# lithium0003/findtextCenterNet

Hardware: AMD Instinct MI355X
Metric: 768x768 images/s (detector fwd+NMS) (higher is better)
Workload: dtype bf16; 1 GPU; BASELINE configs[1]: batch=8/GPU synthetic 768x768x3 uniform-noise tiles, full EfficientNetV2-XL detector forward + NMS + GPU peak decode/100-d gather; global_batch=8, tile=768x768x3, weights=deterministic seed 0 (random-init), parallelism=dp1

## Files before the change

findtextcenternet_amd/csrc/backbone_ops.hip:

```cpp
#include "ftc_common.h"
#include "ftc_host.h"

namespace {

template <typename OutT, typename CopyT, int NQ, bool FAST>
__global__ __launch_bounds__(256) void stem_kernel(const float* __restrict__ in, const float* __restrict__ w,
                                                   const float* __restrict__ bias, OutT* __restrict__ out, CopyT* __restrict__ out2,
                                                   int B, int H, int W, int Ho, int Wo, int C0, int nchw, int act) {
    extern __shared__ __attribute__((aligned(16))) float sw[];
    for (int i = threadIdx.x; i < 27 * C0; i += blockDim.x) sw[i] = w[i];
    __syncthreads();
    const int CG = C0 / (4 * NQ);
    const unsigned total = (unsigned)B * Ho * Wo * CG;
    for (unsigned idx = blockIdx.x * blockDim.x + threadIdx.x; idx < total; idx += gridDim.x * blockDim.x) {
        const unsigned pix = idx / (unsigned)CG;
        const int c0 = (int)(idx - pix * CG) * 4 * NQ;
        const unsigned row = pix / (unsigned)Wo;
        const int ox = (int)(pix - row * Wo);
        const int b = (int)(row / (unsigned)Ho);
        const int oy = (int)(row - (unsigned)b * Ho);
        f32x4 acc[NQ];
#pragma unroll
        for (int q = 0; q < NQ; ++q) acc[q] = *reinterpret_cast<const f32x4*>(bias + c0 + 4 * q);
#pragma unroll
        for (int r = 0; r < 3; ++r) {
            const int iy = oy * 2 - 1 + r;
#pragma unroll
            for (int s = 0; s < 3; ++s) {
                const int ix = ox * 2 - 1 + s;
                if ((unsigned)iy < (unsigned)H && (unsigned)ix < (unsigned)W) {
#pragma unroll
                    for (int c = 0; c < 3; ++c) {
                        const float v = nchw ? in[(((long)b * 3 + c) * H + iy) * W + ix]
                                             : in[(((long)b * H + iy) * W + ix) * 3 + c];
                        const float xv = v * 2.0f - 1.0f;
#pragma unroll
                        for (int q = 0; q < NQ; ++q) acc[q] += xv * *reinterpret_cast<const f32x4*>(sw + ((r * 3 + s) * 3 + c) * C0 + c0 + 4 * q);
                    }
                }
            }
        }
#pragma unroll
        for (int q = 0; q < NQ; ++q) {
            if (act) {
                if constexpr (FAST) acc[q] = act_silu_fast4(acc[q]);
                else {
#pragma unroll
                    for (int e = 0; e < 4; ++e) acc[q][e] = act_silu_precise(acc[q][e]);
                }
            }
            store4<OutT>(out + (long)pix * C0 + c0 + 4 * q, acc[q]);
            if (out2) store4<CopyT>(out2 + (long)pix * C0 + c0 + 4 * q, acc[q]);
        }
    }
}

template <typename T, int STRIDE>
__global__ __launch_bounds__(256) void dwconv_kernel(const T* __restrict__ in, const float* __restrict__ w,
                                                     const float* __restrict__ bias, T* __restrict__ out,
                                                     float* __restrict__ partial, int H, int W, int Ho, int Wo,
                                                     int C, int tilesX, int P, int tiles_per_wg, int act) {
    constexpr int V = 16 / (int)sizeof(T);
    constexpr int LPP = 64 / V;
    constexpr int SLOTS = 256 / LPP;
    constexpr int TH = STRIDE == 1 ? 8 : 4;
    constexpr int TW = 8;
    constexpr int IH = (TH - 1) * STRIDE + 3;
    constexpr int IW = (TW - 1) * STRIDE + 3;
    constexpr int NPX = IH * IW;
    constexpr int NLD = (NPX + SLOTS - 1) / SLOTS;
    __shared__ __attribute__((aligned(16))) T tile[2][NPX * 64];
    __shared__ __attribute__((aligned(16))) float red[SLOTS * 64];

    auto swz = [](int i) { return (STRIDE == 2 && sizeof(T) == 2) ? (i * 64) ^ (((i >> 1) & 1) << 6) : i * 64; };
    const int t = threadIdx.x;
    const int cq = t % LPP;
    const int pt = t / LPP;
    const int c = blockIdx.x * 64 + cq * V;
    const int b = blockIdx.z;
    const bool cok = c < C;
    const int tile0 = blockIdx.y * tiles_per_wg;
    const int ntile = min(tiles_per_wg, P - tile0);

    u32x4 stage[NLD];
    auto fetch = [&](int tileId) {
        const int ty = tileId / tilesX, tx = tileId - ty * tilesX;
        const int iy0 = ty * TH * STRIDE - 1, ix0 = tx * TW * STRIDE - 1;
#pragma unroll
        for (int j = 0; j < NLD; ++j) {
            const int i = pt + j * SLOTS;
            const int ry = i / IW, rx = i - ry * IW;
            const int iy = iy0 + ry, ix = ix0 + rx;
            u32x4 v = {0u, 0u, 0u, 0u};
            if (cok && i < NPX && (unsigned)iy < (unsigned)H && (unsigned)ix < (unsigned)W)
                v = *reinterpret_cast<const u32x4*>(in + (((long)b * H + iy) * W + ix) * C + c);
            stage[j] = v;
        }
    };
    auto commit = [&](int buf) {
#pragma unroll
        for (int j = 0; j < NLD; ++j) {
            const int i = pt + j * SLOTS;
            if (i < NPX) *reinterpret_cast<u32x4*>(&tile[buf][swz(i) + cq * V]) = stage[j];
        }
    };

    fetch(tile0);
    float wv[9][V], bv[V];
#pragma unroll
    for (int e = 0; e < V; ++e) bv[e] = 0.f;
#pragma unroll
    for (int k = 0; k < 9; ++k)
#pragma unroll
        for (int e = 0; e < V; ++e) wv[k][e] = 0.f;
    if (cok) {
#pragma unroll
        for (int k = 0; k < 9; ++k)
#pragma unroll
            for (int q = 0; q < V / 4; ++q) {
                const f32x4 x = *reinterpret_cast<const f32x4*>(w + (long)k * C + c + 4 * q);
#pragma unroll
                for (int e = 0; e < 4; ++e) wv[k][4 * q + e] = x[e];
            }
#pragma unroll
        for (int q = 0; q < V / 4; ++q) {
            const f32x4 x = *reinterpret_cast<const f32x4*>(bias + c + 4 * q);
#pragma unroll
            for (int e = 0; e < 4; ++e) bv[4 * q + e] = x[e];
        }
    }
    commit(0);
    __syncthreads();

    for (int kt = 0; kt < ntile; ++kt) {
        const int tileId = tile0 + kt;
        const int buf = kt & 1;
        if (kt + 1 < ntile) fetch(tileId + 1);
        const int ty = tileId / tilesX, tx = tileId - ty * tilesX;
        const int oy0 = ty * TH, ox0 = tx * TW;
        float sum[V];
#pragma unroll
        for (int e = 0; e < V; ++e) sum[e] = 0.f;
#pragma unroll
        for (int k = 0; k < TH * TW / SLOTS; ++k) {
            const int o = pt + SLOTS * k;
            const int ly = o / TW, lx = o - ly * TW;
            const int oy = oy0 + ly, ox = ox0 + lx;
            float acc[V];
#pragma unroll
            for (int e = 0; e < V; ++e) acc[e] = bv[e];
#pragma unroll
            for (int r = 0; r < 3; ++r)
#pragma unroll
                for (int s = 0; s < 3; ++s) {
                    float x[V];
                    load16<T>(&tile[buf][swz((ly * STRIDE + r) * IW + lx * STRIDE + s) + cq * V], x);
#pragma unroll
                    for (int e = 0; e < V; ++e) acc[e] = fmaf(wv[r * 3 + s][e], x[e], acc[e]);
                }
            if (cok && oy < Ho && ox < Wo) {
                if (act) {
#pragma unroll
                    for (int e = 0; e < V; ++e) acc[e] = sizeof(T) == 2 ? act_silu_fast(acc[e]) : act_silu_precise(acc[e]);
                }
                store16<T>(out + (((long)b * Ho + oy) * Wo + ox) * C + c, acc);
#pragma unroll
                for (int e = 0; e < V; ++e) sum[e] += acc[e];
            }
        }
#pragma unroll
        for (int e = 0; e < V; ++e) red[pt * 64 + cq * V + e] = sum[e];
        if (kt + 1 < ntile) commit(buf ^ 1);
        __syncthreads();
        if (t < 64) {
            float s = 0.f;
#pragma unroll
            for (int k = 0; k < SLOTS; ++k) s += red[k * 64 + t];
            const int cc = blockIdx.x * 64 + t;
            if (cc < C) partial[((long)b * P + tileId) * C + cc] = s;
        }
        __syncthreads();
    }
}

typedef __attribute__((address_space(3))) void lds_ptr_t;
__device__ __forceinline__ void dma16(__amdgpu_buffer_rsrc_t r, lds_ptr_t* dst, int voff) {
    __builtin_amdgcn_raw_ptr_buffer_load_lds(r, dst, 16, voff, 0, 0, 0);
}

template <typename T, bool PRECISE>
__global__ __launch_bounds__(256) void dwconv_strip_kernel(const T* __restrict__ in, const float* __restrict__ w,
                                                           const float* __restrict__ bias, T* __restrict__ out,
                                                           float* __restrict__ partial, int H, int W, int C, int tilesX,
                                                           int P, int tiles_per_wg, int act) {
    constexpr int TH = 8, TW = 8, IW = 10, NPX = 100;
    constexpr int CHS = 16 / (int)sizeof(T);
    constexpr int LPS = 64 / CHS;
    constexpr int PPW = 64 / LPS;
    constexpr int PPP = 4 * PPW;
    constexpr int NLD = (NPX + PPP - 1) / PPP;
    constexpr int OOB = 0x7ffffff0;
    __shared__ __attribute__((aligned(16))) T tile[2][NLD * PPP * 64];
    __shared__ __attribute__((aligned(16))) float red[16 * 64];

    const int t = threadIdx.x;
    const int b = blockIdx.z;
    const int c0 = blockIdx.x * 64;
    const int lane = t & 63, wave = __builtin_amdgcn_readfirstlane(t >> 6);
    const __amdgpu_buffer_rsrc_t rin = __builtin_amdgcn_make_buffer_rsrc(const_cast<T*>(in + (long)b * H * W * C), 0,
                                                                         H * W * C * (int)sizeof(T), 0x00020000);
    const int s_px = wave * PPW + lane / LPS;
    const int s_coff = (c0 + (lane % LPS) * CHS < C) ? (c0 + (lane % LPS) * CHS) * (int)sizeof(T) : OOB;
    const int cq = t & 15, col = (t >> 4) & 7, rh = t >> 7;
    const int c = c0 + cq * 4;
    const bool cok = c < C;
    const int tile0 = blockIdx.y * tiles_per_wg;
    const int ntile = min(tiles_per_wg, P - tile0);

    auto issue = [&](int tileId, int buf) {
        const int ty = tileId / tilesX, tx = tileId - ty * tilesX;
        const int iy0 = ty * TH - 1, ix0 = tx * TW - 1;
#pragma unroll
        for (int j = 0; j < NLD; ++j) {
            const int i = s_px + j * PPP;
            const int ry = i / IW, rx = i - ry * IW;
            const int iy = iy0 + ry, ix = ix0 + rx;
            const bool ok = i < NPX && (unsigned)iy < (unsigned)H && (unsigned)ix < (unsigned)W;
            dma16(rin, (lds_ptr_t*)&tile[buf][(j * PPP + wave * PPW) * 64], ok ? (iy * W + ix) * C * (int)sizeof(T) + s_coff : OOB);
        }
    };

    issue(tile0, 0);
    f32x4 wv[9], bv = {0.f, 0.f, 0.f, 0.f};
#pragma unroll
    for (int k = 0; k < 9; ++k) wv[k] = bv;
    if (cok) {
#pragma unroll
        for (int k = 0; k < 9; ++k) wv[k] = *reinterpret_cast<const f32x4*>(w + (long)k * C + c);
        bv = *reinterpret_cast<const f32x4*>(bias + c);
    }

    f32x4 sum = {0.f, 0.f, 0.f, 0.f};
    for (int kt = 0; kt < ntile; ++kt) {
        const int tileId = tile0 + kt;
        const int buf = kt & 1;
        asm volatile("s_waitcnt vmcnt(0)" ::: "memory");
        __syncthreads();
        if (kt + 1 < ntile) issue(tileId + 1, buf ^ 1);
        const int ty = tileId / tilesX, tx = tileId - ty * tilesX;
        const int oy0 = ty * TH + rh * 4, ox = tx * TW + col;
        f32x4 acc[4] = {bv, bv, bv, bv};
        const T* tp = &tile[buf][((rh * 4) * IW + col) * 64 + cq * 4];
#pragma unroll
        for (int r = 0; r < 6; ++r) {
            f32x4 x[3];
#pragma unroll
            for (int s2 = 0; s2 < 3; ++s2) x[s2] = load4<T>(tp + (r * IW + s2) * 64);
#pragma unroll
            for (int oo = 0; oo < 4; ++oo) {
                const int kr = r - oo;
                if (kr >= 0 && kr < 3) {
#pragma unroll
                    for (int s2 = 0; s2 < 3; ++s2)
#pragma unroll
                        for (int e = 0; e < 4; ++e) acc[oo][e] = fmaf(wv[kr * 3 + s2][e], x[s2][e], acc[oo][e]);
                }
            }
        }
#pragma unroll
        for (int oo = 0; oo < 4; ++oo) {
            const int oy = oy0 + oo;
            if (cok && oy < H && ox < W) {
                if (!PRECISE || act) {
#pragma unroll
                    for (int e = 0; e < 4; ++e) acc[oo][e] = PRECISE ? act_silu_precise(acc[oo][e]) : act_silu_fast(acc[oo][e]);
                }
                store4<T>(out + (((long)b * H + oy) * W + ox) * C + c, acc[oo]);
                sum += acc[oo];
            }
        }
    }
    *reinterpret_cast<f32x4*>(&red[(t >> 4) * 64 + cq * 4]) = sum;
    __syncthreads();
    if (t < 64 && c0 + t < C) {
        float s2 = 0.f;
#pragma unroll
        for (int k = 0; k < 16; ++k) s2 += red[k * 64 + t];
        float* pp = partial + ((long)b * P + tile0) * C + c0 + t;
        pp[0] = s2;
        for (int kt = 1; kt < ntile; ++kt) pp[(long)kt * C] = 0.f;
    }
}

__global__ __launch_bounds__(512) void se_fc1_kernel(const float* __restrict__ partial, const float* __restrict__ w1,
                                                     const float* __restrict__ b1, float* __restrict__ hidden,
                                                     int C, int S, int P, float inv_hw) {
    extern __shared__ __attribute__((aligned(16))) float mean[];
    const int b = blockIdx.y;
    const int t = threadIdx.x;
    const int CQ = C >> 2;
    const int lane = t & 63, wave = t >> 6;
    const int sidx = blockIdx.x * 8 + wave;
    constexpr int WMAX = 15;
    f32x4 wv[WMAX];
    const f32x4* wr = reinterpret_cast<const f32x4*>(w1 + (long)(sidx < S ? sidx : 0) * C);
#pragma unroll
    for (int i = 0; i < WMAX; ++i) {
        const int q = lane + 64 * i;
        wv[i] = q < CQ ? wr[q] : f32x4{0.f, 0.f, 0.f, 0.f};
    }
    const f32x4* pb = reinterpret_cast<const f32x4*>(partial + (long)b * P * C);
    for (int q = t; q < CQ; q += 512) {
        f32x4 s = {0.f, 0.f, 0.f, 0.f};
#pragma unroll 4
        for (int p = 0; p < P; ++p) s += pb[(long)p * CQ + q];
        reinterpret_cast<f32x4*>(mean)[q] = s * inv_hw;
    }
    __syncthreads();
    if (sidx >= S) return;
    f32x4 acc = {0.f, 0.f, 0.f, 0.f};
#pragma unroll
    for (int i = 0; i < WMAX; ++i) {
        const int q = lane + 64 * i;
        if (q < CQ) acc += wv[i] * reinterpret_cast<const f32x4*>(mean)[q];
    }
    for (int q = lane + 64 * WMAX; q < CQ; q += 64) acc += wr[q] * reinterpret_cast<const f32x4*>(mean)[q];
    float a = wave_sum((acc[0] + acc[1]) + (acc[2] + acc[3]));
    if (lane == 0) hidden[(long)b * S + sidx] = act_silu_precise(a + b1[sidx]);
}

__device__ __forceinline__ void se_load_hidden(float* hid, const float* __restrict__ hidden, const float* __restrict__ hpart,
                                               const float* __restrict__ b1, int b, int S, int NS, int t, int nthreads) {
    if (hpart) {
        const float* hp = hpart + (long)b * NS * S;
        for (int s = t; s < S; s += nthreads) {
            float a0 = 0.f, a1 = 0.f, a2 = 0.f, a3 = 0.f;
            int j = 0;
            for (; j + 4 <= NS; j += 4) {
                a0 += hp[(long)j * S + s];
                a1 += hp[(long)(j + 1) * S + s];
                a2 += hp[(long)(j + 2) * S + s];
                a3 += hp[(long)(j + 3) * S + s];
            }
            for (; j < NS; ++j) a0 += hp[(long)j * S + s];
            hid[s] = act_silu_precise(((a0 + a1) + (a2 + a3)) + b1[s]);
        }
    } else {
        for (int s = t; s < S; s += nthreads) hid[s] = hidden[(long)b * S + s];
    }
}

template <bool FOLD, typename T>
__global__ __launch_bounds__(256) void se_fc2_kernel(const float* __restrict__ hidden, const float* __restrict__ w2t,
                                                     const float* __restrict__ b2, float* __restrict__ scale, int C, int S,
                                                     const T* __restrict__ wp, T* __restrict__ wb, int N,
                                                     const float* __restrict__ hpart, const float* __restrict__ b1, int NS) {
    extern __shared__ __attribute__((aligned(16))) float hid[];
    const int b = blockIdx.y;
    se_load_hidden(hid, hidden, hpart, b1, b, S, NS, threadIdx.x, 256);
    __syncthreads();
    const int c = blockIdx.x * 256 + threadIdx.x;
    float sc = 0.f;
    if (c < C) {
        float acc = b2[c];
#pragma unroll 8
        for (int s = 0; s < S; ++s) acc += hid[s] * w2t[(long)s * C + c];
        sc = sigmoid_precise(acc);
        if (!FOLD || blockIdx.z == 0) scale[(long)b * C + c] = sc;
    }
    if constexpr (FOLD) {
        float* lsc = hid + S;
        lsc[threadIdx.x] = sc;
        __syncthreads();
        const int chunk = threadIdx.x & 31, r0 = threadIdx.x >> 5;
        const int cc = blockIdx.x * 256 + chunk * 8;
        if (cc >= C) return;
        float f[8];
#pragma unroll
        for (int e = 0; e < 8; ++e) f[e] = lsc[chunk * 8 + e];
        const int rows = (N + gridDim.z - 1) / gridDim.z;
        const int n_lo = blockIdx.z * rows, n_hi = min(N, n_lo + rows);
        T* dst = wb + (long)b * N * C;
#pragma unroll 4
        for (int n = n_lo + r0; n < n_hi; n += 8) {
            float x[8];
            load16<T>(wp + (long)n * C + cc, x);
#pragma unroll
            for (int e = 0; e < 8; ++e) x[e] *= f[e];
            store16<T>(dst + (long)n * C + cc, x);
        }
    }
}


template <typename T>
__global__ __launch_bounds__(256) void se_fc2_fold64_kernel(const float* __restrict__ hidden, const float* __restrict__ w2t,
                                                            const float* __restrict__ b2, float* __restrict__ scale, int C, int S,
                                                            const T* __restrict__ wp, T* __restrict__ wb, int N,
                                                            const float* __restrict__ hpart, const float* __restrict__ b1, int NS) {
    extern __shared__ __attribute__((aligned(16))) float lds_f[];
    float* hid = lds_f;
    float* part = lds_f + ((S + 3) & ~3);
    float* lsc = part + 256;
    const int b = blockIdx.y, t = threadIdx.x;
    const int cl = t & 63, sg = t >> 6;
    const int c = blockIdx.x * 64 + cl;
    const int s_lo = sg * ((S + 3) / 4), s_hi = min(S, s_lo + (S + 3) / 4);
    constexpr int SMAX = 40;
    float wreg[SMAX];
#pragma unroll
    for (int i = 0; i < SMAX; ++i) wreg[i] = (c < C && s_lo + i < s_hi) ? w2t[(long)(s_lo + i) * C + c] : 0.f;
    se_load_hidden(hid, hidden, hpart, b1, b, S, NS, t, 256);
    __syncthreads();
    float acc = 0.f;
#pragma unroll
    for (int i = 0; i < SMAX; ++i)
        if (s_lo + i < s_hi) acc += hid[s_lo + i] * wreg[i];
    for (int s = s_lo + SMAX; s < s_hi; ++s) acc += hid[s] * w2t[(long)s * C + c];
    part[sg * 64 + cl] = acc;
    __syncthreads();
    if (t < 64) {
        float sc = 0.f;
        if (c < C) {
            sc = sigmoid_precise(b2[c] + ((part[cl] + part[64 + cl]) + (part[128 + cl] + part[192 + cl])));
            if (blockIdx.z == 0) scale[(long)b * C + c] = sc;
        }
        lsc[cl] = sc;
    }
    __syncthreads();
    const int chunk = t & 7, r0 = t >> 3;
    const int cc = blockIdx.x * 64 + chunk * 8;
    if (cc >= C) return;
    float f[8];
#pragma unroll
    for (int e = 0; e < 8; ++e) f[e] = lsc[chunk * 8 + e];
    const int rows = (N + gridDim.z - 1) / gridDim.z;
    const int n_lo = blockIdx.z * rows, n_hi = min(N, n_lo + rows);
    T* dst = wb + (long)b * N * C;
#pragma unroll 4
    for (int n = n_lo + r0; n < n_hi; n += 32) {
        float x[8];
        load16<T>(wp + (long)n * C + cc, x);
#pragma unroll
        for (int e = 0; e < 8; ++e) x[e] *= f[e];
        store16<T>(dst + (long)n * C + cc, x);
    }
}

__global__ __launch_bounds__(256) void se_fc2_foldx3_kernel(const float* __restrict__ hidden, const float* __restrict__ w2t,
                                                            const float* __restrict__ b2, float* __restrict__ scale, int C, int S,
                                                            const u32x4* __restrict__ wp, u32x4* __restrict__ wb, int N,
                                                            const float* __restrict__ hpart, const float* __restrict__ b1, int NS) {
    extern __shared__ __attribute__((aligned(16))) float lds_f[];
    float* hid = lds_f;
    float* part = lds_f + ((S + 3) & ~3);
    float* lsc = part + 256;
    const int b = blockIdx.y, t = threadIdx.x;
    const int cl = t & 63, sg = t >> 6;
    const int c = blockIdx.x * 64 + cl;
    const int s_lo = sg * ((S + 3) / 4), s_hi = min(S, s_lo + (S + 3) / 4);
    constexpr int SMAX = 40;
    float wreg[SMAX];
#pragma unroll
    for (int i = 0; i < SMAX; ++i) wreg[i] = (c < C && s_lo + i < s_hi) ? w2t[(long)(s_lo + i) * C + c] : 0.f;
    se_load_hidden(hid, hidden, hpart, b1, b, S, NS, t, 256);
    __syncthreads();
    float acc = 0.f;
#pragma unroll
    for (int i = 0; i < SMAX; ++i)
        if (s_lo + i < s_hi) acc += hid[s_lo + i] * wreg[i];
    for (int s = s_lo + SMAX; s < s_hi; ++s) acc += hid[s] * w2t[(long)s * C + c];
    part[sg * 64 + cl] = acc;
    __syncthreads();
    if (t < 64) {
        float sc = 0.f;
        if (c < C) {
            sc = sigmoid_precise(b2[c] + ((part[cl] + part[64 + cl]) + (part[128 + cl] + part[192 + cl])));
            if (blockIdx.z == 0) scale[(long)b * C + c] = sc;
        }
        lsc[cl] = sc;
    }
    __syncthreads();
    const int chunk = t & 15, r0 = t >> 4;
    const int cc = blockIdx.x * 64 + chunk * 4;
    if (cc >= C) return;
    float f[4];
#pragma unroll
    for (int e = 0; e < 4; ++e) f[e] = lsc[chunk * 4 + e];
    const int rows = (N + gridDim.z - 1) / gridDim.z;
    const int n_lo = blockIdx.z * rows, n_hi = min(N, n_lo + rows);
    u32x4* dst = wb + (long)b * N * (C >> 2);
#pragma unroll 4
    for (int n = n_lo + r0; n < n_hi; n += 16) {
        const u32x4 v = wp[(long)n * (C >> 2) + (cc >> 2)];
        typedef _Float16 h4 __attribute__((ext_vector_type(4)));
        const u32x2 hu = {v[0], v[1]}, lu = {v[2], v[3]};
        const h4 hi = __builtin_bit_cast(h4, hu), lo = __builtin_bit_cast(h4, lu);
        h4 oh, ol;
#pragma unroll
        for (int e = 0; e < 4; ++e) {
            const float x = f16_sat(((float)hi[e] + (float)lo[e]) * f[e]);
            const _Float16 hh = (_Float16)x;
            oh[e] = hh;
            ol[e] = (_Float16)(x - (float)hh);
        }
        const u32x2 ohu = __builtin_bit_cast(u32x2, oh), olu = __builtin_bit_cast(u32x2, ol);
        dst[(long)n * (C >> 2) + (cc >> 2)] = u32x4{ohu[0], ohu[1], olu[0], olu[1]};
    }
}

}

hipError_t launch_stem(const OpArgs& a, hipStream_t s) {
    const ftc_op& o = *a.op;
    const bool wide = o.Cout % 16 == 0;
    const long total = (long)o.B * o.Ho * o.Wo * (o.Cout / (wide ? 16 : 4));
    const int blocks = (int)((total + 255) / 256 < 16384 ? (total + 255) / 256 : 16384);
    const size_t lds = (size_t)27 * o.Cout * sizeof(float);
    const int nchw = (o.flags & FTC_FLAG_IN_NCHW) ? 1 : 0;
    const int act = o.act != FTC_ACT_NONE ? 1 : 0;
#define STEM_LAUNCH(OT, CT, NQ, FAST)                                                                                                        \
    hipLaunchKernelGGL((stem_kernel<OT, CT, NQ, FAST>), dim3(blocks), dim3(256), lds, s, (const float*)a.in, (const float*)a.w, a.bias, (OT*)a.out, \
                       (CT*)a.out2, o.B, o.H, o.W, o.Ho, o.Wo, o.Cout, nchw, act)
#define STEM_WIDTH(OT, CT, FAST) do { if (wide) STEM_LAUNCH(OT, CT, 4, FAST); else STEM_LAUNCH(OT, CT, 1, FAST); } while (0)
    if (o.out_dtype == FTC_F32 && o.w_dtype == FTC_F16) STEM_WIDTH(float, _Float16, true);
    else if (o.out_dtype == FTC_F32 && a.out2) STEM_WIDTH(float, __bf16, true);
    else if (o.out_dtype == FTC_F32) STEM_WIDTH(float, __bf16, false);
    else if (o.out_dtype == FTC_F16) STEM_WIDTH(_Float16, _Float16, true);
    else STEM_WIDTH(__bf16, __bf16, true);
#undef STEM_WIDTH
#undef STEM_LAUNCH
    return hipGetLastError();
}

bool ftc_dwconv_strip(const ftc_op& o) { return o.stride == 1 && !(o.flags & 0x100) && (ftc_is16(o.in_dtype) ? o.act != FTC_ACT_NONE : (o.Cin % 4 == 0)); }

hipError_t launch_dwconv(const OpArgs& a, hipStream_t s) {
    const ftc_op& o = *a.op;
    const int TH = o.stride == 1 ? 8 : 4, TW = 8;
    const int tilesX = (o.Wo + TW - 1) / TW, tilesY = (o.Ho + TH - 1) / TH;
    const int P = tilesX * tilesY;
    if (P != o.aux0) return hipErrorInvalidValue;
    const bool strip = ftc_dwconv_strip(o);
    const long slabs = (long)((o.Cin + 63) / 64) * o.B;
    const long slots = 256L * (strip ? (o.in_dtype == FTC_F32 ? 2 : 4) : o.in_dtype == FTC_F32 ? 3 : 2);
    int tpw = 1;
    long best = -1;
    for (int cand = 1; cand <= (P < 16 ? P : 16); ++cand) {
        const long wgs = slabs * ((P + cand - 1) / cand);
        const long cost = ((wgs + slots - 1) / slots) * cand;
        if (best < 0 || cost <= best) { best = cost; tpw = cand; }
    }
    dim3 grid((o.Cin + 63) / 64, (P + tpw - 1) / tpw, o.B);
#define DW_LAUNCH(T, ST)                                                                                      \
    hipLaunchKernelGGL((dwconv_kernel<T, ST>), grid, dim3(256), 0, s, (const T*)a.in, (const float*)a.w, a.bias, \
                       (T*)a.out, a.aux, o.H, o.W, o.Ho, o.Wo, o.Cin, tilesX, P, tpw, o.act != FTC_ACT_NONE ? 1 : 0)
    const int act = o.act != FTC_ACT_NONE ? 1 : 0;
    if (strip && o.in_dtype == FTC_F32)
        hipLaunchKernelGGL((dwconv_strip_kernel<float, true>), grid, dim3(256), 0, s, (const float*)a.in, (const float*)a.w, a.bias,
                           (float*)a.out, a.aux, o.H, o.W, o.Cin, tilesX, P, tpw, act);
    else if (o.in_dtype == FTC_F32) { if (o.stride == 1) DW_LAUNCH(float, 1); else DW_LAUNCH(float, 2); }
    else if (strip && o.in_dtype == FTC_F16)
        hipLaunchKernelGGL((dwconv_strip_kernel<_Float16, false>), grid, dim3(256), 0, s, (const _Float16*)a.in, (const float*)a.w, a.bias,
                           (_Float16*)a.out, a.aux, o.H, o.W, o.Cin, tilesX, P, tpw, act);
    else if (strip)
        hipLaunchKernelGGL((dwconv_strip_kernel<__bf16, false>), grid, dim3(256), 0, s, (const __bf16*)a.in, (const float*)a.w, a.bias,
                           (__bf16*)a.out, a.aux, o.H, o.W, o.Cin, tilesX, P, tpw, act);
    else if (o.in_dtype == FTC_F16) { if (o.stride == 1) DW_LAUNCH(_Float16, 1); else DW_LAUNCH(_Float16, 2); }
    else { if (o.stride == 1) DW_LAUNCH(__bf16, 1); else DW_LAUNCH(__bf16, 2); }
#undef DW_LAUNCH
    return hipGetLastError();
}

hipError_t launch_se(const OpArgs& a, hipStream_t s) {
    const ftc_op& o = *a.op;
    const int C = o.Cin, S = o.aux0, P = o.aux1;
    float* hidden = const_cast<float*>(static_cast<const float*>(a.in2));
    const bool hp = (o.flags & FTC_FLAG_SE_HPART) != 0;
    const float* hpart = hp ? a.aux : nullptr;
    if (!hp) {
        hipLaunchKernelGGL(se_fc1_kernel, dim3((S + 7) / 8, o.B), dim3(512), (size_t)C * sizeof(float), s, (const float*)a.aux,
                           (const float*)a.w, a.bias, hidden, C, S, P, 1.0f / (float)(o.H * o.W));
        hipError_t e = hipGetLastError();
        if (e != hipSuccess) return e;
    }
    if (hp && (o.flags & FTC_FLAG_SE_FOLD) && (o.flags & 0x100)) return hipErrorInvalidValue;
    if ((o.flags & FTC_FLAG_SE_FOLD) && o.w_dtype == FTC_F32) {
        const int cb = (C + 63) / 64;
        int nz = (768 + cb * o.B - 1) / (cb * o.B);
        const int max_nz = (o.Cout_total + 15) / 16;
        nz = nz < 1 ? 1 : nz > max_nz ? max_nz : nz;
        hipLaunchKernelGGL(se_fc2_foldx3_kernel, dim3(cb, o.B, nz), dim3(256), (size_t)(((S + 3) & ~3) + 256 + 64) * sizeof(float), s, hidden,
                           (const float*)a.w2, a.bias2, (float*)a.out, C, S, (const u32x4*)a.in, (u32x4*)a.out2, o.Cout_total, hpart, a.bias, P);
    } else if ((o.flags & FTC_FLAG_SE_FOLD) && !(o.flags & 0x100)) {
        const int cb = (C + 63) / 64;
        int nz = (768 + cb * o.B - 1) / (cb * o.B);
        const int max_nz = (o.Cout_total + 31) / 32;
        nz = nz < 1 ? 1 : nz > max_nz ? max_nz : nz;
        if (o.w_dtype == FTC_F16)
            hipLaunchKernelGGL(se_fc2_fold64_kernel<_Float16>, dim3(cb, o.B, nz), dim3(256), (size_t)(((S + 3) & ~3) + 256 + 64) * sizeof(float), s, hidden,
                               (const float*)a.w2, a.bias2, (float*)a.out, C, S, (const _Float16*)a.in, (_Float16*)a.out2, o.Cout_total, hpart, a.bias, P);
        else
            hipLaunchKernelGGL(se_fc2_fold64_kernel<__bf16>, dim3(cb, o.B, nz), dim3(256), (size_t)(((S + 3) & ~3) + 256 + 64) * sizeof(float), s, hidden,
                               (const float*)a.w2, a.bias2, (float*)a.out, C, S, (const __bf16*)a.in, (__bf16*)a.out2, o.Cout_total, hpart, a.bias, P);
    } else if (o.flags & FTC_FLAG_SE_FOLD) {
        const int cb = (C + 255) / 256;
        int nz = 512 / (cb * o.B);
        nz = nz < 1 ? 1 : nz > 8 ? 8 : nz;
        if (o.w_dtype == FTC_F16)
            hipLaunchKernelGGL((se_fc2_kernel<true, _Float16>), dim3(cb, o.B, nz), dim3(256), (size_t)(S + 256) * sizeof(float), s, hidden,
                               (const float*)a.w2, a.bias2, (float*)a.out, C, S, (const _Float16*)a.in, (_Float16*)a.out2, o.Cout_total, nullptr, nullptr, 0);
        else
            hipLaunchKernelGGL((se_fc2_kernel<true, __bf16>), dim3(cb, o.B, nz), dim3(256), (size_t)(S + 256) * sizeof(float), s, hidden,
                               (const float*)a.w2, a.bias2, (float*)a.out, C, S, (const __bf16*)a.in, (__bf16*)a.out2, o.Cout_total, nullptr, nullptr, 0);
    } else if (hp && C % 64 == 0 && S <= 160) {
        hipLaunchKernelGGL(se_fc2_fold64_kernel<__bf16>, dim3(C / 64, o.B, 1), dim3(256), (size_t)(((S + 3) & ~3) + 256 + 64) * sizeof(float), s, hidden,
                           (const float*)a.w2, a.bias2, (float*)a.out, C, S, (const __bf16*)nullptr, (__bf16*)nullptr, 0, hpart, a.bias, P);
    } else {
        hipLaunchKernelGGL((se_fc2_kernel<false, __bf16>), dim3((C + 255) / 256, o.B), dim3(256), (size_t)S * sizeof(float), s, hidden,
                           (const float*)a.w2, a.bias2, (float*)a.out, C, S, (const __bf16*)nullptr, (__bf16*)nullptr, 0, hpart, a.bias, P);
    }
    return hipGetLastError();
}
```

Baseline: 684.5 images/s.

## Prefetch fold weights and stage SE hidden partials via buffer-to-LDS loads

Rewrites the SE fc2+weight-fold kernels around a shared helper. The first group of weight rows for the fold is loaded into registers before the gate computation, so that memory latency overlaps the gate math. When they fit, the hidden partial sums are staged into LDS with buffer_load_lds and reduced in parallel, replacing the per-thread se_load_hidden path. The remaining rows are processed in register batches of 10. This raises register pressure and LDS use, which may lower occupancy in exchange for better latency hiding.

```diff
diff --git a/findtextcenternet_amd/csrc/backbone_ops.hip b/findtextcenternet_amd/csrc/backbone_ops.hip
--- a/findtextcenternet_amd/csrc/backbone_ops.hip
+++ b/findtextcenternet_amd/csrc/backbone_ops.hip
@@ -393,58 +393,175 @@
 }
 
 
+constexpr int SE_SMAX = 40;
+constexpr int SE_HP_SLOTS = 48;
+constexpr int SE_FOLD_G = 10;
+__host__ __device__ inline bool se_hpart_staged(int S, int P) { return S <= 4 * SE_SMAX && (long)P * S <= 256L * SE_HP_SLOTS; }
+inline size_t se_gates64_lds(int S, int P, bool hp) {
+    const int S4 = (S + 3) & ~3;
+    return (size_t)(S4 + 256 + 64 + (hp && se_hpart_staged(S, P) ? ((P * S + 255) & ~255) + 4 * S4 : 0)) * sizeof(float);
+}
+
+template <int G>
+__device__ __forceinline__ void se_gates64(const float* __restrict__ hidden, const float* __restrict__ w2t, const float* __restrict__ b2,
+                                           float* __restrict__ scale, int C, int S, const float* __restrict__ hpart,
+                                           const float* __restrict__ b1, int NS, float* lds_f, const u32x4* __restrict__ wrow,
+                                           long rstep, int nrows, int nrmax, u32x4 (&pre)[G]) {
+    const int S4 = (S + 3) & ~3;
+    float* hid = lds_f;
+    float* part = lds_f + S4;
+    float* lsc = part + 256;
+    float* stage = lsc + 64;
+    const int b = blockIdx.y, t = threadIdx.x;
+    const int cl = t & 63, sg = __builtin_amdgcn_readfirstlane(t >> 6);
+    const int c = blockIdx.x * 64 + cl;
+    const int s_lo = sg * ((S + 3) / 4), s_hi = min(S, s_lo + (S + 3) / 4);
+    const int nst = hpart && se_hpart_staged(S, NS) ? NS * S : 0;
+    if (nst) {
+        const __amdgpu_buffer_rsrc_t rhp = __builtin_amdgcn_make_buffer_rsrc(const_cast<float*>(hpart + (long)b * nst), 0, nst * (int)sizeof(float), 0x00020000);
+#pragma unroll 2
+        for (int o = 0; o < nst; o += 256)
+            __builtin_amdgcn_raw_ptr_buffer_load_lds(rhp, (lds_ptr_t*)&stage[o + 64 * sg], 4, (t + o) * (int)sizeof(float), 0, 0, 0);
+    }
+    const int tc = min(t, S - 1);
+    const float b1v = hpart ? b1[tc] : 0.f;
+    const float h0 = hpart ? 0.f : hidden[(long)b * S + tc];
+    const int cq = min(c, C - 1);
+    float wreg[SE_SMAX];
+#pragma unroll
+    for (int i = 0; i < SE_SMAX; ++i) wreg[i] = s_lo + i < s_hi ? w2t[(long)(s_lo + i) * C + cq] : 0.f;
+    const float b2v = b2[cq];
+#pragma unroll
+    for (int i = 0; i < G; ++i) pre[i] = i < nrmax ? wrow[min(i, nrows - 1) * rstep] : u32x4{0u, 0u, 0u, 0u};
+    if (nst) {
+        asm volatile("s_waitcnt vmcnt(0)" ::: "memory");
+        __syncthreads();
+        float* acc4 = stage + ((nst + 255) & ~255);
+        const int m4 = NS & ~3;
+#pragma unroll
+        for (int i = 0; i < 3; ++i) {
+            const int q = t + 256 * i;
+            if (q < 4 * S) {
+                const int k = (q >= S) + (q >= 2 * S) + (q >= 3 * S), s = q - k * S;
+                float a = 0.f;
+#pragma unroll 8
+                for (int j = k; j < m4; j += 4) a += stage[j * S + s];
+                if (k == 0)
+                    for (int j = m4; j < NS; ++j) a += stage[j * S + s];
+                acc4[k * S4 + s] = a;
+            }
+        }
+        __syncthreads();
+        if (t < S) hid[t] = act_silu_precise(((acc4[t] + acc4[S4 + t]) + (acc4[2 * S4 + t] + acc4[3 * S4 + t])) + b1v);
+    } else if (hpart) {
+        se_load_hidden(hid, hidden, hpart, b1, b, S, NS, t, 256);
+    } else {
+        if (t < S) hid[t] = h0;
+        for (int s = t + 256; s < S; s += 256) hid[s] = hidden[(long)b * S + s];
+    }
+    __syncthreads();
+    float acc = 0.f;
+#pragma unroll
+    for (int i = 0; i < SE_SMAX; ++i)
+        if (s_lo + i < s_hi) acc += hid[s_lo + i] * wreg[i];
+    for (int s = s_lo + SE_SMAX; s < s_hi; ++s) acc += hid[s] * w2t[(long)s * C + cq];
+    part[sg * 64 + cl] = acc;
+    __syncthreads();
+    if (t < 64) {
+        float sc = 0.f;
+        if (c < C) {
+            sc = sigmoid_precise(b2v + ((part[cl] + part[64 + cl]) + (part[128 + cl] + part[192 + cl])));
+            if (blockIdx.z == 0) scale[(long)b * C + c] = sc;
+        }
+        lsc[cl] = sc;
+    }
+    __syncthreads();
+}
+
+template <typename T> __device__ __forceinline__ u32x4 se_fold_chunk(u32x4 v, const float (&f)[8]) {
+    float x[8];
+    if constexpr (__is_same(T, __bf16)) {
+#pragma unroll
+        for (int e = 0; e < 4; ++e) {
+            x[2 * e] = __uint_as_float(v[e] << 16);
+            x[2 * e + 1] = __uint_as_float(v[e] & 0xffff0000u);
+        }
+        bf16x8 o;
+#pragma unroll
+        for (int e = 0; e < 8; ++e) o[e] = (__bf16)(x[e] * f[e]);
+        return __builtin_bit_cast(u32x4, o);
+    } else {
+        const f16x8 h = __builtin_bit_cast(f16x8, v);
+        f16x8 o;
+#pragma unroll
+        for (int e = 0; e < 8; ++e) o[e] = (_Float16)f16_sat((float)h[e] * f[e]);
+        return __builtin_bit_cast(u32x4, o);
+    }
+}
+__device__ __forceinline__ u32x4 se_fold_chunk_x3(u32x4 v, const float (&f)[4]) {
+    const u32x2 hu = {v[0], v[1]}, lu = {v[2], v[3]};
+    const f16x4 hi = __builtin_bit_cast(f16x4, hu), lo = __builtin_bit_cast(f16x4, lu);
+    f16x4 oh, ol;
+#pragma unroll
+    for (int e = 0; e < 4; ++e) {
+        const float x = f16_sat(((float)hi[e] + (float)lo[e]) * f[e]);
+        const _Float16 hh = (_Float16)x;
+        oh[e] = hh;
+        ol[e] = (_Float16)(x - (float)hh);
+    }
+    const u32x2 ohu = __builtin_bit_cast(u32x2, oh), olu = __builtin_bit_cast(u32x2, ol);
+    return u32x4{ohu[0], ohu[1], olu[0], olu[1]};
+}
+
+template <int EPC, typename FoldFn>
+__device__ __forceinline__ void se_gates_fold64(const float* __restrict__ hidden, const float* __restrict__ w2t, const float* __restrict__ b2,
+                                                float* __restrict__ scale, int C, int S, const u32x4* __restrict__ wp, u32x4* __restrict__ wb,
+                                                int N, const float* __restrict__ hpart, const float* __restrict__ b1, int NS, float* lds_f,
+                                                FoldFn fold) {
+    constexpr int G = SE_FOLD_G, LPR = 64 / EPC, RPP = 256 / LPR;
+    const int t = threadIdx.x;
+    const int chunk = t & (LPR - 1), r0 = t / LPR;
+    const int cc = blockIdx.x * 64 + chunk * EPC;
+    const int rows = (N + gridDim.z - 1) / gridDim.z;
+    const int n_lo = blockIdx.z * rows, n_hi = min(N, n_lo + rows);
+    const int n0 = n_lo + r0;
+    const int nrows = (cc < C && n0 < n_hi) ? (n_hi - n0 + RPP - 1) / RPP : 0;
+    const int nrmax = n_lo < n_hi ? (n_hi - n_lo + RPP - 1) / RPP : 0;
+    const long cu = C / EPC, first = (long)n0 * cu + cc / EPC, rstep = (long)RPP * cu;
+    const u32x4* wrow = wp + first;
+    u32x4 va[G];
+    se_gates64<G>(hidden, w2t, b2, scale, C, S, hpart, b1, NS, lds_f, nrows ? wrow : wp + ((long)n_lo * cu + blockIdx.x * (64 / EPC)), rstep,
+                  max(nrows, 1), nrmax, va);
+    if (nrows == 0) return;
+    const float* lsc = lds_f + ((S + 3) & ~3) + 256;
+    float f[EPC];
+#pragma unroll
+    for (int e = 0; e < EPC; ++e) f[e] = lsc[chunk * EPC + e];
+    u32x4* drow = wb + (long)blockIdx.y * N * cu + first;
+    auto request = [&](u32x4 (&v)[G], int g) {
+#pragma unroll
+        for (int i = 0; i < G; ++i) v[i] = wrow[min(g + i, nrows - 1) * rstep];
+    };
+    auto finish = [&](const u32x4 (&v)[G], int g) {
+#pragma unroll
+        for (int i = 0; i < G; ++i)
+            if (g + i < nrows) drow[(g + i) * rstep] = fold(v[i], f);
+    };
+    finish(va, 0);
+    for (int g = G; g < nrmax; g += G) {
+        request(va, g);
+        finish(va, g);
+    }
+}
+
 template <typename T>
 __global__ __launch_bounds__(256) void se_fc2_fold64_kernel(const float* __restrict__ hidden, const float* __restrict__ w2t,
                                                             const float* __restrict__ b2, float* __restrict__ scale, int C, int S,
                                                             const T* __restrict__ wp, T* __restrict__ wb, int N,
                                                             const float* __restrict__ hpart, const float* __restrict__ b1, int NS) {
     extern __shared__ __attribute__((aligned(16))) float lds_f[];
-    float* hid = lds_f;
-    float* part = lds_f + ((S + 3) & ~3);
-    float* lsc = part + 256;
-    const int b = blockIdx.y, t = threadIdx.x;
-    const int cl = t & 63, sg = t >> 6;
-    const int c = blockIdx.x * 64 + cl;
-    const int s_lo = sg * ((S + 3) / 4), s_hi = min(S, s_lo + (S + 3) / 4);
-    constexpr int SMAX = 40;
-    float wreg[SMAX];
-#pragma unroll
-    for (int i = 0; i < SMAX; ++i) wreg[i] = (c < C && s_lo + i < s_hi) ? w2t[(long)(s_lo + i) * C + c] : 0.f;
-    se_load_hidden(hid, hidden, hpart, b1, b, S, NS, t, 256);
-    __syncthreads();
-    float acc = 0.f;
-#pragma unroll
-    for (int i = 0; i < SMAX; ++i)
-        if (s_lo + i < s_hi) acc += hid[s_lo + i] * wreg[i];
-    for (int s = s_lo + SMAX; s < s_hi; ++s) acc += hid[s] * w2t[(long)s * C + c];
-    part[sg * 64 + cl] = acc;
-    __syncthreads();
-    if (t < 64) {
-        float sc = 0.f;
-        if (c < C) {
-            sc = sigmoid_precise(b2[c] + ((part[cl] + part[64 + cl]) + (part[128 + cl] + part[192 + cl])));
-            if (blockIdx.z == 0) scale[(long)b * C + c] = sc;
-        }
-        lsc[cl] = sc;
-    }
-    __syncthreads();
-    const int chunk = t & 7, r0 = t >> 3;
-    const int cc = blockIdx.x * 64 + chunk * 8;
-    if (cc >= C) return;
-    float f[8];
-#pragma unroll
-    for (int e = 0; e < 8; ++e) f[e] = lsc[chunk * 8 + e];
-    const int rows = (N + gridDim.z - 1) / gridDim.z;
-    const int n_lo = blockIdx.z * rows, n_hi = min(N, n_lo + rows);
-    T* dst = wb + (long)b * N * C;
-#pragma unroll 4
-    for (int n = n_lo + r0; n < n_hi; n += 32) {
-        float x[8];
-        load16<T>(wp + (long)n * C + cc, x);
-#pragma unroll
-        for (int e = 0; e < 8; ++e) x[e] *= f[e];
-        store16<T>(dst + (long)n * C + cc, x);
-    }
+    se_gates_fold64<8>(hidden, w2t, b2, scale, C, S, reinterpret_cast<const u32x4*>(wp), reinterpret_cast<u32x4*>(wb), N, hpart, b1, NS, lds_f,
+                       [](u32x4 v, const float (&f)[8]) { return se_fold_chunk<T>(v, f); });
 }
 
 __global__ __launch_bounds__(256) void se_fc2_foldx3_kernel(const float* __restrict__ hidden, const float* __restrict__ w2t,
@@ -452,61 +569,8 @@
                                                             const u32x4* __restrict__ wp, u32x4* __restrict__ wb, int N,
                                                             const float* __restrict__ hpart, const float* __restrict__ b1, int NS) {
     extern __shared__ __attribute__((aligned(16))) float lds_f[];
-    float* hid = lds_f;
-    float* part = lds_f + ((S + 3) & ~3);
-    float* lsc = part + 256;
-    const int b = blockIdx.y, t = threadIdx.x;
-    const int cl = t & 63, sg = t >> 6;
-    const int c = blockIdx.x * 64 + cl;
-    const int s_lo = sg * ((S + 3) / 4), s_hi = min(S, s_lo + (S + 3) / 4);
-    constexpr int SMAX = 40;
-    float wreg[SMAX];
-#pragma unroll
-    for (int i = 0; i < SMAX; ++i) wreg[i] = (c < C && s_lo + i < s_hi) ? w2t[(long)(s_lo + i) * C + c] : 0.f;
-    se_load_hidden(hid, hidden, hpart, b1, b, S, NS, t, 256);
-    __syncthreads();
-    float acc = 0.f;
-#pragma unroll
-    for (int i = 0; i < SMAX; ++i)
-        if (s_lo + i < s_hi) acc += hid[s_lo + i] * wreg[i];
-    for (int s = s_lo + SMAX; s < s_hi; ++s) acc += hid[s] * w2t[(long)s * C + c];
-    part[sg * 64 + cl] = acc;
-    __syncthreads();
-    if (t < 64) {
-        float sc = 0.f;
-        if (c < C) {
-            sc = sigmoid_precise(b2[c] + ((part[cl] + part[64 + cl]) + (part[128 + cl] + part[192 + cl])));
-            if (blockIdx.z == 0) scale[(long)b * C + c] = sc;
-        }
-        lsc[cl] = sc;
-    }
-    __syncthreads();
-    const int chunk = t & 15, r0 = t >> 4;
-    const int cc = blockIdx.x * 64 + chunk * 4;
-    if (cc >= C) return;
-    float f[4];
-#pragma unroll
-    for (int e = 0; e < 4; ++e) f[e] = lsc[chunk * 4 + e];
-    const int rows = (N + gridDim.z - 1) / gridDim.z;
-    const int n_lo = blockIdx.z * rows, n_hi = min(N, n_lo + rows);
-    u32x4* dst = wb + (long)b * N * (C >> 2);
-#pragma unroll 4
-    for (int n = n_lo + r0; n < n_hi; n += 16) {
-        const u32x4 v = wp[(long)n * (C >> 2) + (cc >> 2)];
-        typedef _Float16 h4 __attribute__((ext_vector_type(4)));
-        const u32x2 hu = {v[0], v[1]}, lu = {v[2], v[3]};
-        const h4 hi = __builtin_bit_cast(h4, hu), lo = __builtin_bit_cast(h4, lu);
-        h4 oh, ol;
-#pragma unroll
-        for (int e = 0; e < 4; ++e) {
-            const float x = f16_sat(((float)hi[e] + (float)lo[e]) * f[e]);
-            const _Float16 hh = (_Float16)x;
-            oh[e] = hh;
-            ol[e] = (_Float16)(x - (float)hh);
-        }
-        const u32x2 ohu = __builtin_bit_cast(u32x2, oh), olu = __builtin_bit_cast(u32x2, ol);
-        dst[(long)n * (C >> 2) + (cc >> 2)] = u32x4{ohu[0], ohu[1], olu[0], olu[1]};
-    }
+    se_gates_fold64<4>(hidden, w2t, b2, scale, C, S, wp, wb, N, hpart, b1, NS, lds_f,
+                       [](u32x4 v, const float (&f)[4]) { return se_fold_chunk_x3(v, f); });
 }
 
 }
@@ -590,7 +654,7 @@
         int nz = (768 + cb * o.B - 1) / (cb * o.B);
         const int max_nz = (o.Cout_total + 15) / 16;
         nz = nz < 1 ? 1 : nz > max_nz ? max_nz : nz;
-        hipLaunchKernelGGL(se_fc2_foldx3_kernel, dim3(cb, o.B, nz), dim3(256), (size_t)(((S + 3) & ~3) + 256 + 64) * sizeof(float), s, hidden,
+        hipLaunchKernelGGL(se_fc2_foldx3_kernel, dim3(cb, o.B, nz), dim3(256), se_gates64_lds(S, P, hp), s, hidden,
                            (const float*)a.w2, a.bias2, (float*)a.out, C, S, (const u32x4*)a.in, (u32x4*)a.out2, o.Cout_total, hpart, a.bias, P);
     } else if ((o.flags & FTC_FLAG_SE_FOLD) && !(o.flags & 0x100)) {
         const int cb = (C + 63) / 64;
@@ -598,10 +662,10 @@
         const int max_nz = (o.Cout_total + 31) / 32;
         nz = nz < 1 ? 1 : nz > max_nz ? max_nz : nz;
         if (o.w_dtype == FTC_F16)
-            hipLaunchKernelGGL(se_fc2_fold64_kernel<_Float16>, dim3(cb, o.B, nz), dim3(256), (size_t)(((S + 3) & ~3) + 256 + 64) * sizeof(float), s, hidden,
+            hipLaunchKernelGGL(se_fc2_fold64_kernel<_Float16>, dim3(cb, o.B, nz), dim3(256), se_gates64_lds(S, P, hp), s, hidden,
                                (const float*)a.w2, a.bias2, (float*)a.out, C, S, (const _Float16*)a.in, (_Float16*)a.out2, o.Cout_total, hpart, a.bias, P);
         else
-            hipLaunchKernelGGL(se_fc2_fold64_kernel<__bf16>, dim3(cb, o.B, nz), dim3(256), (size_t)(((S + 3) & ~3) + 256 + 64) * sizeof(float), s, hidden,
+            hipLaunchKernelGGL(se_fc2_fold64_kernel<__bf16>, dim3(cb, o.B, nz), dim3(256), se_gates64_lds(S, P, hp), s, hidden,
                                (const float*)a.w2, a.bias2, (float*)a.out, C, S, (const __bf16*)a.in, (__bf16*)a.out2, o.Cout_total, hpart, a.bias, P);
     } else if (o.flags & FTC_FLAG_SE_FOLD) {
         const int cb = (C + 255) / 256;
@@ -614,7 +678,7 @@
             hipLaunchKernelGGL((se_fc2_kernel<true, __bf16>), dim3(cb, o.B, nz), dim3(256), (size_t)(S + 256) * sizeof(float), s, hidden,
                                (const float*)a.w2, a.bias2, (float*)a.out, C, S, (const __bf16*)a.in, (__bf16*)a.out2, o.Cout_total, nullptr, nullptr, 0);
     } else if (hp && C % 64 == 0 && S <= 160) {
-        hipLaunchKernelGGL(se_fc2_fold64_kernel<__bf16>, dim3(C / 64, o.B, 1), dim3(256), (size_t)(((S + 3) & ~3) + 256 + 64) * sizeof(float), s, hidden,
+        hipLaunchKernelGGL(se_fc2_fold64_kernel<__bf16>, dim3(C / 64, o.B, 1), dim3(256), se_gates64_lds(S, P, hp), s, hidden,
                            (const float*)a.w2, a.bias2, (float*)a.out, C, S, (const __bf16*)nullptr, (__bf16*)nullptr, 0, hpart, a.bias, P);
     } else {
         hipLaunchKernelGGL((se_fc2_kernel<false, __bf16>), dim3((C + 255) / 256, o.B), dim3(256), (size_t)S * sizeof(float), s, hidden,
```

Result: no change. 690.2 images/s, median of 6 (+0.8%).
